# HAHHHD/mllp

Measured on AMD Instinct MI355X. Metric: LP instances/sec (fwd+bwd) on Netlib batch; achieved HBM GB/s on CSR SpMM, higher is better.
Workload: dtype f32; 1 GPU; netlib_full: BASELINE.json configs[2], 97 instances / 1,074,147 nnz per global batch, one block-diagonal batch per GPU, one Adam step per global batch: fwd + BCE + bwd + gradient all-reduce + Adam, fp32; global_batch=97, instances_rank0=97, nnz_rank0=1074147, hip_graph=False, parallelism=dp1

## Files before the change

### mllp_amd/csrc/fused_kernels.hip

```cpp
#include <algorithm>
#include <vector>

#include "device_utils.h"
#include "host_graph.h"
#include "internal.h"
#include "node_bodies.h"

namespace mllp {

typedef float f32x4m __attribute__((ext_vector_type(4)));

#ifdef MLLP_TIMING_BUILD
static int g_fused_abl = [] {
    const char* e = getenv("MLLP_FUSED_ABL");
    return e ? atoi(e) : 0;
}();
#define FUSED_ABL(bit) ((J.abl & (bit)) != 0)
__device__ unsigned long long g_fused_stamps[8192 * 8];
__device__ unsigned long long g_fused_stamps1[8192 * 8];
#define FUSED_STAMP(k)                                                                      \
    {                                                                                       \
        __builtin_amdgcn_sched_barrier(0);                                                  \
        const unsigned long long now_ = __builtin_amdgcn_s_memtime();                       \
        __builtin_amdgcn_sched_barrier(0);                                                  \
// ... 1293 lines not shown
    const int tid = threadIdx.x, lane = tid & 63, wave = tid >> 6;
    for (int j = 0; j < A.n_jobs; ++j) {
        const BwdJob1& J = A.job[j];
        BwdW1& W = Ws_[j];
        if (tid < 16) { W.wv[tid] = J.p.Wv[tid]; W.bv[tid] = J.p.bv[tid]; W.we[tid] = J.p.we[tid]; }
        if (tid == 0) { W.pq = J.D[OFF_PQ]; W.pq0 = J.D[OFF_PQ0]; W.pt = J.D[OFF_PT]; W.pt0 = J.D[OFF_PT0]; }
    }
    __syncthreads();
    float* tiles = tiles_ + wave * TILE1;
    const int px = blockIdx.x % NP, bi = blockIdx.x / NP, gp = gridDim.x / NP;
    const int gw = bi * FW + wave;
#ifdef MLLP_TIMING_BUILD
    unsigned long long stamp_sum[8] = {0, 0, 0, 0, 0, 0, 0, 0};
    unsigned long long stamp_last = __builtin_amdgcn_s_memtime();
    const unsigned long long stamp_begin = stamp_last;
#define STAMP_ARGS1 , stamp_sum, stamp_last
#else
#define STAMP_ARGS1
#endif
    for (int j = 0; j < A.n_jobs; ++j) {
        const BwdJob1& J = A.job[j];
        const PartTiers P = J.s.part[px];
        f32x4m accT = splat4(0.0f);
        float accS[6] = {0.0f, 0.0f, 0.0f, 0.0f, 0.0f, 0.0f};
        for (int k = bi; k < P.n_block; k += gp)
            bwd1_row(J, Ws_[j], block_slot<1>(J.s, P.row0 + k, tid), lane, merge_lds, tiles, accT, accS STAMP_ARGS1);
        WaveList wl = wave_list(J.s, px, gw);
        for (int c0 = 0; c0 < wl.L; c0 += 64) {
            wave_list_chunk(wl, c0, lane);
            int it = wave_list_get(wl, 0);
            SlotReq q = item_request<1>(J.s, P, max(it, 0), lane);
            for (int k = 0; it >= 0; ++k) {
                const int itn = wave_list_get(wl, k + 1);
                const RowSlot r = slot_make(q);
                q = item_request<1>(J.s, P, max(itn, 0), lane);
                bwd1_row(J, Ws_[j], r, lane, merge_lds, tiles, accT, accS STAMP_ARGS1);
#ifdef MLLP_TIMING_BUILD
                stamp_sum[7] += 1;
#endif
                it = itn;
            }
        }
        __syncthreads();
        float* red = tiles_;
#pragma unroll
        for (int q = 0; q < 4; ++q) red[wave * 262 + ((lane >> 4) * 4 + q) * 16 + (lane & 15)] = accT[q];
#pragma unroll
        for (int i = 0; i < 6; ++i) {
            const float v = wave_sum(accS[i]);
            if (lane == 0) red[wave * 262 + 256 + i] = v;
        }
        __syncthreads();
        float* dst = J.stats + (size_t)blockIdx.x * STAT_FLOATS;
        for (int i = tid; i < STAT_FLOATS; i += FT) dst[i] = 0.0f;
        __syncthreads();
        if (tid < 262) {
            float v = 0.0f;
            for (int w = 0; w < FW; ++w) v += red[w * 262 + tid];
            const int o = tid >> 4, n = tid & 15;
            if (tid >= 256) {
                const int i = tid - 256;
                const int slot = i == 0 ? 768 : i == 1 ? 1024 : i == 2 ? 1280 : i == 3 ? 1280 + 16 : i == 4 ? 1536 : 1536 + 16;
                dst[slot] = v;
            } else if (n == 0) dst[o * 16] = v;
            else if (n == 1) dst[256 + o * 16] = v;
            else if (n < 5) dst[512 + o * 16 + (n - 2)] = v;
        }
        __syncthreads();
#ifdef MLLP_TIMING_BUILD
        stamp_last = __builtin_amdgcn_s_memtime();
#endif
    }
#ifdef MLLP_TIMING_BUILD
    if (lane == 0) {
        stamp_sum[6] = __builtin_amdgcn_s_memtime() - stamp_begin;
        unsigned long long* d = g_fused_stamps1 + (size_t)(blockIdx.x * FW + wave) * 8;
        for (int k = 0; k < 8; ++k) d[k] = stamp_sum[k];
    }
#endif
#undef STAMP_ARGS1
}

__global__ __launch_bounds__(RT) void fused_head_bwd_kernel(int n, const float* __restrict__ h3, const float* __restrict__ fcw,
                                                            const float* __restrict__ dlogits, const int* __restrict__ perm,
                                                            float* __restrict__ dh3, float* __restrict__ head_part) {
    __shared__ float head_lds[(RT / 64) * 18];
    const int tid = threadIdx.x, lane = tid & 63, part = lane & 3;
    HeadAcc ha;
    ha.w = f4zero(); ha.b = 0.0f; ha.l = 0.0f;
    const float4 fw = ld4(fcw + 4 * part);
    for (int row = blockIdx.x * (RT / 4) + (tid >> 2); row < n; row += gridDim.x * (RT / 4)) {
        const float dz = dlogits[perm[row]];
        const float4 hv = ld4(h3 + (size_t)row * 16 + 4 * part);
        *reinterpret_cast<float4*>(dh3 + (size_t)row * 16 + 4 * part) = f4scale(fw, dz);
        fma4(dz, hv, ha.w);
        if (part == 0) ha.b += dz;
    }
    head_partials_store<RT / 64>(ha, head_lds, head_part, tid);
}

struct ReduceArgs {
    const float* stats[MODEL_CONVS];
    float* out[MODEL_CONVS];
    int nblk;
    const float* head_part;
    float* head_out;
    float* loss_out;
};

__device__ __forceinline__ void fused_reduce_body(const ReduceArgs& A, int n_conv) {
    __shared__ float sh[32][32];
    const int tid = threadIdx.x;
    if ((int)blockIdx.x == n_conv * STAT_TILES) {
        if (!A.head_part) return;
        const int col = tid & 31, slice = tid >> 5;
        float v = 0.0f;
        if (col < 18)
            for (int b = slice; b < A.nblk; b += 32) v += A.head_part[(size_t)b * 18 + col];
        sh[slice][col] = v;
        __syncthreads();
        if (tid < 18) {
            float t = 0.0f;
            for (int q = 0; q < 32; ++q) t += sh[q][tid];
            if (tid < 17) A.head_out[tid] = t;
            else if (A.loss_out) A.loss_out[0] = t;
        }
        return;
    }
    float* sh4 = &sh[0][0];
    const int col = tid & 255, slice = tid >> 8;
    const int c = blockIdx.x / STAT_TILES, tile = blockIdx.x % STAT_TILES;
    const float* src = A.stats[c] + tile * 256 + col;
    float v = 0.0f;
    int b = slice;
    for (; b + 124 < A.nblk; b += 128) {
        float t[32];
#pragma unroll
        for (int q = 0; q < 32; ++q) t[q] = src[(size_t)(b + 4 * q) * STAT_FLOATS];
#pragma unroll
        for (int q = 0; q < 32; ++q) v += t[q];
    }
    for (; b + 28 < A.nblk; b += 32) {
        float t[8];
#pragma unroll
        for (int q = 0; q < 8; ++q) t[q] = src[(size_t)(b + 4 * q) * STAT_FLOATS];
#pragma unroll
        for (int q = 0; q < 8; ++q) v += t[q];
    }
    for (; b < A.nblk; b += 4) v += src[(size_t)b * STAT_FLOATS];
    sh4[slice * 256 + col] = v;
    __syncthreads();
    if (tid < 256) A.out[c][tile * 256 + tid] = (sh4[tid] + sh4[256 + tid]) + (sh4[512 + tid] + sh4[768 + tid]);
}
__global__ __launch_bounds__(RT) void fused_reduce_kernel(ReduceArgs A, int n_conv) { fused_reduce_body(A, n_conv); }

struct TailArgs {
    ReduceArgs R;
    ConvParams p[MODEL_CONVS];
    int cin[MODEL_CONVS];
    float* grads[MODEL_CONVS];
    float* zero;
    int n_zero;
    float* params; const float* grads_all; float* m; float* v; float* state;
    float eps;
    int n_params;
    float* D[MODEL_CONVS];
    unsigned long long* sync;
    unsigned* err;
};
__device__ __forceinline__ bool tail_barrier(unsigned long long* cnt, unsigned long long target, unsigned* err_host) {
    __shared__ int ok_s;
    unsigned long long* err_dev = cnt + 2;
    __syncthreads();
    if (threadIdx.x == 0) {
        __threadfence();
        __hip_atomic_fetch_add(cnt, 1ull, __ATOMIC_RELEASE, __HIP_MEMORY_SCOPE_AGENT);
        int spins = 0;
        while (__hip_atomic_load(cnt, __ATOMIC_ACQUIRE, __HIP_MEMORY_SCOPE_AGENT) < target && ++spins < (1 << 22))
            __builtin_amdgcn_s_sleep(8);
        if (spins >= (1 << 22)) {
            __hip_atomic_store(err_dev, 1ull, __ATOMIC_RELAXED, __HIP_MEMORY_SCOPE_AGENT);
            __hip_atomic_store(err_host, 1u, __ATOMIC_RELAXED, __HIP_MEMORY_SCOPE_SYSTEM);
        }
        __threadfence();
        ok_s = __hip_atomic_load(err_dev, __ATOMIC_RELAXED, __HIP_MEMORY_SCOPE_AGENT) == 0ull;
    }
    __syncthreads();
    return ok_s != 0;
}
__global__ __launch_bounds__(RT) void fused_tail_kernel(TailArgs A, int n_conv) {
    const unsigned long long G = gridDim.x, epoch = A.sync[1];
    const int b = blockIdx.x;
    const float step = A.state[0] + 1.0f, lr = A.state[1], b1 = A.state[2], b2 = A.state[3];
    fused_reduce_body(A.R, n_conv);
    if (!tail_barrier(A.sync, (epoch + 1) * G, A.err)) return;
    if (b < n_conv) {
        finalize_conv_body(A.cin[b], A.p[b], A.R.out[b], 1, A.grads[b]);
        __syncthreads();
        const int off = (int)(A.grads[b] - A.grads_all), n = 4 * FEAT * A.cin[b] + 5 * FEAT;
        adam_slice(A.params + off, A.grads_all + off, A.m + off, A.v + off, step, lr, b1, b2, A.eps, 1.0f, n);
        __syncthreads();
        if (threadIdx.x < BLOCK) param_prep_body(A.p[b], A.cin[b], A.D[b]);
    } else if (b == n_conv) {
        for (int k = threadIdx.x; k < A.n_zero; k += RT) A.zero[k] = 0.0f;
        const int off = (int)(A.R.head_out - A.grads_all);
        adam_slice(A.params + off, A.grads_all + off, A.m + off, A.v + off, step, lr, b1, b2, A.eps, 1.0f, A.n_params - off);
        if (threadIdx.x == 0) {
            A.state[0] = step;
            A.sync[1] = epoch + 1;
        }
    }
}

__global__ __launch_bounds__(256) void fused_fill_kernel(int n_dst, const int* __restrict__ perm, const int* __restrict__ ptr,
                                                         const int* __restrict__ idx, const float* __restrict__ val,
                                                         const int* __restrict__ inv_src, const int* __restrict__ sptr,
                                                         int2* __restrict__ sent) {
    const int k = blockIdx.x * 4 + (threadIdx.x >> 6), lane = threadIdx.x & 63;
    if (k >= n_dst) return;
    const int r = perm[k], beg = ptr[r], deg = ptr[r + 1] - beg, o = sptr[k];
    for (int e = lane; e < deg; e += 64) sent[o + e] = make_int2(inv_src[idx[beg + e]], __float_as_int(val[beg + e]));
}
__global__ void fused_permute_kernel(int n, const int* __restrict__ perm, const float* __restrict__ src, float* __restrict__ dst) {
    for (int i = blockIdx.x * blockDim.x + threadIdx.x; i < n; i += gridDim.x * blockDim.x) dst[i] = src[perm[i]];
}
__global__ void fused_pregather_kernel(int64_t nnz, const int2* __restrict__ sent, const float* __restrict__ xs,
                                       float2* __restrict__ sax) {
    for (int64_t e = blockIdx.x * (int64_t)blockDim.x + threadIdx.x; e < nnz; e += (int64_t)gridDim.x * blockDim.x) {
        const int2 v = sent[e];
        sax[e] = make_float2(__int_as_float(v.y), xs[v.x]);
    }
}

#ifdef MLLP_TIMING_BUILD
extern "C" int mllp_timing_read_stamps(unsigned long long* host, int n) {
    return hipMemcpyFromSymbol(host, HIP_SYMBOL(g_fused_stamps), (size_t)n * sizeof(unsigned long long)) == hipSuccess ? 0 : -1;
}
extern "C" int mllp_timing_read_stamps1(unsigned long long* host, int n) {
    return hipMemcpyFromSymbol(host, HIP_SYMBOL(g_fused_stamps1), (size_t)n * sizeof(unsigned long long)) == hipSuccess ? 0 : -1;
}
#endif

template <class T>
static int dev_alloc(mllp_graph* g, size_t count, T** out, const T* host = nullptr, size_t room = 1) {
    void* p = nullptr;
    MLLP_HIP_TRY(hipMalloc(&p, std::max<size_t>(count, room) * sizeof(T)));
    if (count < room) MLLP_HIP_TRY(hipMemset(p, 0, room * sizeof(T)));
    g->allocs.push_back(p);
    if (host && count) MLLP_HIP_TRY(hipMemcpy(p, host, count * sizeof(T), hipMemcpyHostToDevice));
    *out = static_cast<T*>(p);
    return MLLP_OK;
}

static void set_tiers(FusedTiersDev& d, const FusedTiers& t) {
    d.n_block = t.n_block; d.n_wave = t.n_wave; d.n_group = t.n_group; d.n_base = t.n_base;
}

int fused_refill_values(mllp_graph* g, hipStream_t s) {
    int rc;
    if (g->M > 0) {
        hipLaunchKernelGGL(fused_fill_kernel, dim3((unsigned)((g->M + 3) / 4)), dim3(256), 0, s, (int)g->M, g->perm_c, g->A.ptr,
                           g->A.idx, g->A.val, g->inv_v, g->FA.sptr, reinterpret_cast<int2*>(g->FA.sent));
        if ((rc = check_launch("fused_fill A"))) return rc;
    }
    if (g->N > 0) {
        hipLaunchKernelGGL(fused_fill_kernel, dim3((unsigned)((g->N + 3) / 4)), dim3(256), 0, s, (int)g->N, g->perm_v, g->At.ptr,
                           g->At.idx, g->At.val, g->inv_c, g->FAt.sptr, reinterpret_cast<int2*>(g->FAt.sent));
        if ((rc = check_launch("fused_fill At"))) return rc;
    }
    return MLLP_OK;
}

int fused_graph_build(mllp_graph* g, const int* h_csr_ptr, const int* h_csc_ptr) {
    if (g->fused_built) return MLLP_OK;
    if ((int64_t)g->h_csr_ptr.size() != g->M + 1 && !h_csr_ptr) return fail(MLLP_EINVAL, "fused path: no host row pointers");
    HostFusedOrient hc, hv;
    {
#ifdef MLLP_SCALAR_PARTITION
        const std::vector<int> part = host_partition_instances(host_instance_cost(h_csr_ptr, g->h_inst_ptr_m),
                                                               host_instance_cost(h_csc_ptr, g->h_inst_ptr_n), FUSED_PARTS);
#else
        const std::vector<int> part = host_partition_instances_v(host_instance_loads(h_csr_ptr, g->h_inst_ptr_m),
                                                                 host_instance_loads(h_csc_ptr, g->h_inst_ptr_n), FUSED_PARTS);
#endif
        host_build_fused_orient(h_csr_ptr, (int)g->M, g->h_inst_ptr_m, part, &hc);
        host_build_fused_orient(h_csc_ptr, (int)g->N, g->h_inst_ptr_n, part, &hv);
    }
    int rc;
    if ((rc = dev_alloc(g, (size_t)g->M, &g->perm_c, hc.perm.data()))) return rc;
    if ((rc = dev_alloc(g, (size_t)g->N, &g->perm_v, hv.perm.data()))) return rc;
    if ((rc = dev_alloc(g, (size_t)g->M, &g->inv_c, hc.inv.data()))) return rc;
    if ((rc = dev_alloc(g, (size_t)g->N, &g->inv_v, hv.inv.data()))) return rc;
    FusedOrient& A = g->FA;
    FusedOrient& At = g->FAt;
    A.n_dst = (int)g->M; A.n_src = (int)g->N; A.nnz = (int)g->nnz;
    At.n_dst = (int)g->N; At.n_src = (int)g->M; At.nnz = (int)g->nnz;
    for (int q = 0; q < NP; ++q) {
        set_tiers(A.t16[q], hc.t16[q]); set_tiers(A.t1[q], hc.t1[q]);
        set_tiers(At.t16[q], hv.t16[q]); set_tiers(At.t1[q], hv.t1[q]);
    }
    for (int q = 0; q <= NP; ++q) { A.row0[q] = hc.row0[q]; At.row0[q] = hv.row0[q]; }
    {
        const int gp = fused_grid(g) / NP;
        const HostFusedOrient* ho[2] = {&hc, &hv};
        FusedOrient* dv[2] = {&A, &At};
        for (int k = 0; k < 2; ++k) {
            HostWaveLists l16, l16x2, l1;
            host_build_wave_lists(*ho[k], false, gp * FW, FW, 4, &l16);
            host_build_wave_lists(*ho[k], false, 2 * gp * FW, FW, 2, &l16x2);
            host_build_wave_lists(*ho[k], true, gp * FW, FW, 8, &l1);
            FusedOrient& d = *dv[k];
            d.L16 = l16.L; d.nw16 = l16.waves_per_part;
            d.L16x2 = l16x2.L; d.nw16x2 = l16x2.waves_per_part;
            d.L1 = l1.L; d.nw1 = l1.waves_per_part;
            if ((rc = dev_alloc(g, l16.order.size(), &d.lst16, l16.order.data()))) return rc;
            if ((rc = dev_alloc(g, l16x2.order.size(), &d.lst16x2, l16x2.order.data()))) return rc;
            if ((rc = dev_alloc(g, l1.order.size(), &d.lst1, l1.order.data()))) return rc;
        }
    }
    if ((rc = dev_alloc(g, (size_t)g->M + 1, &A.sptr, hc.sptr.data(), 2))) return rc;
    if ((rc = dev_alloc(g, (size_t)g->N + 1, &At.sptr, hv.sptr.data(), 2))) return rc;
    if ((rc = dev_alloc(g, (size_t)g->nnz * 2, &A.sent, (const int*)nullptr, 2))) return rc;
    if ((rc = dev_alloc(g, (size_t)g->nnz * 2, &At.sent, (const int*)nullptr, 2))) return rc;
    if ((rc = dev_alloc(g, (size_t)g->nnz * 2, &A.sax, (const float*)nullptr, 2))) return rc;
    if ((rc = dev_alloc(g, (size_t)g->nnz * 2, &At.sax, (const float*)nullptr, 2))) return rc;
    if ((rc = dev_alloc(g, (size_t)g->N, &g->inv_n_p))) return rc;
    if ((rc = dev_alloc(g, (size_t)g->N, &g->x1_p))) return rc;
    if ((rc = dev_alloc(g, (size_t)g->M, &g->x2_p))) return rc;
    if ((rc = dev_alloc(g, (size_t)g->N, &g->labels_p))) return rc;
    if (!g->tail_sync) {
        if ((rc = dev_alloc(g, (size_t)4, &g->tail_sync))) return rc;
        MLLP_HIP_TRY(hipMemset(g->tail_sync, 0, 32));
        MLLP_HIP_TRY(hipHostMalloc((void**)&g->tail_err_host, 64, hipHostMallocMapped));
        *g->tail_err_host = 0u;
        MLLP_HIP_TRY(hipHostGetDevicePointer((void**)&g->tail_err_dev, g->tail_err_host, 0));
    }
    if ((rc = fused_refill_values(g, 0))) return rc;
    if (g->N > 0) {
        hipLaunchKernelGGL(fused_permute_kernel, dim3(256), dim3(256), 0, 0, (int)g->N, g->perm_v, g->inv_n, g->inv_n_p);
        if ((rc = check_launch("fused_permute inv_n"))) return rc;
    }
    MLLP_HIP_TRY(hipDeviceSynchronize());
    g->fused_built = true;
    return MLLP_OK;
}

int fused_bind(mllp_graph* g, const float* x1, const float* x2, const float* labels, hipStream_t s) {
    int rc;
    hipStreamCaptureStatus cap = hipStreamCaptureStatusNone;
    (void)hipStreamIsCapturing(s, &cap);
    const bool capturing = cap != hipStreamCaptureStatusNone;
    if (capturing) g->bound_x1 = g->bound_x2 = g->bound_labels = nullptr;
    if (x1 != g->bound_x1 || x2 != g->bound_x2) {
        if (g->N > 0) hipLaunchKernelGGL(fused_permute_kernel, dim3(256), dim3(256), 0, s, (int)g->N, g->perm_v, x1, g->x1_p);
        if (g->M > 0) hipLaunchKernelGGL(fused_permute_kernel, dim3(256), dim3(256), 0, s, (int)g->M, g->perm_c, x2, g->x2_p);
        if (g->nnz > 0) {
            hipLaunchKernelGGL(fused_pregather_kernel, dim3(1024), dim3(256), 0, s, g->nnz,
                               reinterpret_cast<const int2*>(g->FA.sent), g->x1_p, reinterpret_cast<float2*>(g->FA.sax));
            hipLaunchKernelGGL(fused_pregather_kernel, dim3(1024), dim3(256), 0, s, g->nnz,
                               reinterpret_cast<const int2*>(g->FAt.sent), g->x2_p, reinterpret_cast<float2*>(g->FAt.sax));
        }
        if ((rc = check_launch("fused_bind inputs"))) return rc;
        if (!capturing) { g->bound_x1 = x1; g->bound_x2 = x2; }
    }
    if (labels && labels != g->bound_labels) {
        if (g->N > 0) hipLaunchKernelGGL(fused_permute_kernel, dim3(256), dim3(256), 0, s, (int)g->N, g->perm_v, labels, g->labels_p);
        if ((rc = check_launch("fused_bind labels"))) return rc;
        if (!capturing) g->bound_labels = labels;
    }
    return MLLP_OK;
}

int fused_grid(const mllp_graph* g) { return std::max(std::min(g->n_cu, STAT_BLOCKS_MAX) / NP, 1) * NP; }

static FwdJob16 fwd_job16(const FusedOrient& o, const FusedModel& m, int c, const float* x_src, const float* x_dst, float* h) {
    const ConvWs& w = m.w.c[c];
    FwdJob16 J = {};
    J.s = items_dev(o, 0);
    J.x_src = x_src; J.x_dst = x_dst; J.D = w.derived; J.p = conv_params_at(conv_at(m.P, c), MODEL_CONV[c].cin);
    J.h = h; J.Z = w.Z; J.aux = w.aux;
    J.head = 0;
#ifdef MLLP_TIMING_BUILD
    J.abl = g_fused_abl;
#endif
    return J;
}
static FwdJob1 fwd_job1(const FusedOrient& o, const FusedModel& m, int c, const float* x_dst, float* h) {
    const ConvWs& w = m.w.c[c];
    FwdJob1 J = {};
    J.s = items_dev(o, 1);
    J.x_dst = x_dst; J.D = w.derived; J.p = conv_params_at(conv_at(m.P, c), MODEL_CONV[c].cin);
    J.h = h; J.Z = w.Z; J.aux = w.aux;
    return J;
}

int fused_forward(mllp_graph* g, const FusedModel& m, int head_mode, hipStream_t s, bool skip_prep) {
    const int G = fused_grid(g);
    const ModelWs& w = m.w;
    int rc;
    if ((rc = fused_bind(g, m.x1, m.x2, head_mode == 2 ? m.labels : nullptr, s))) return rc;
    if (!skip_prep && (rc = model_param_prep(m.P, w, s))) return rc;
    {
        FwdLaunch1 L = {};
        L.n_jobs = 2;
        L.job[0] = fwd_job1(g->FAt, m, CONV_1V, g->x1_p, w.h1v);
        L.job[1] = fwd_job1(g->FA, m, CONV_1C, g->x2_p, w.h1c);
        hipLaunchKernelGGL(fused_fwd1_kernel, dim3(G), dim3(FT), 0, s, L);
        if ((rc = check_launch("fused_fwd1"))) return rc;
    }
    {
        FwdLaunch16 L = {};
        L.n_jobs = 2;
        L.job[0] = fwd_job16(g->FAt, m, CONV_2V, w.h1c, w.h1v, w.h2v);
        L.job[1] = fwd_job16(g->FA, m, CONV_2C, w.h1v, w.h1c, w.h2c);
        L.job[0].perm = g->perm_v; L.job[1].perm = g->perm_c;
        hipLaunchKernelGGL(fused_fwd16_kernel, dim3(G), dim3(FT), 0, s, L);
        if ((rc = check_launch("fused_fwd16 layer 2"))) return rc;
    }
    {
        FwdLaunch16 L = {};
        L.n_jobs = 1;
        L.job[0] = fwd_job16(g->FAt, m, CONV_3V, w.h2c, w.h2v, w.h3v);
        FwdJob16& J = L.job[0];
        J.head = head_mode;
        J.fcw = m.P + OFF_FC; J.fcb = m.P + OFF_FC + FEAT; J.inv_n = g->inv_n_p; J.labels = g->labels_p; J.perm = g->perm_v;
        J.inv_batch = m.inv_batch;
        J.logits = m.logits; J.g_out = w.d3v; J.head_part = w.head_partials;
        hipLaunchKernelGGL(fused_fwd16_kernel, dim3(G), dim3(FT), 0, s, L);
        if ((rc = check_launch("fused_fwd16 layer 3"))) return rc;
    }
    return MLLP_OK;
}

int fused_head_backward(const mllp_graph* g, const FusedModel& m, const float* dlogits, hipStream_t s) {
    const int G = fused_grid(g);
    hipLaunchKernelGGL(fused_head_bwd_kernel, dim3(G), dim3(RT), 0, s, (int)g->N, m.w.h3v, m.P + OFF_FC, dlogits, g->perm_v,
                       m.w.d3v, m.w.head_partials);
    return check_launch("fused_head_bwd");
}

static BwdJob16 bwd_job16(const FusedOrient& o, const FusedModel& m, int c, const float* x_src, const float* x_dst,
                          const float* h, const float* dh_a, const float* dh_b, float* dx_dst, bool need_rec, bool mask_dx) {
    const ConvWs& w = m.w.c[c];
    BwdJob16 J = {};
    J.s = items_dev(o, 0);
    J.x_src = x_src; J.x_dst = x_dst; J.D = w.derived; J.p = conv_params_at(conv_at(m.P, c), MODEL_CONV[c].cin);
    J.h = h; J.dh_a = dh_a; J.dh_b = dh_b; J.Z = w.Z; J.aux = w.aux;
    J.rec = need_rec ? w.rec : nullptr;
    J.dx_dst = dx_dst;
    J.mask_dx = mask_dx ? 1 : 0;
    J.stats = w.stats;
#ifdef MLLP_TIMING_BUILD
    J.abl = g_fused_abl;
#endif
    return J;
}
static SrcJob16 src_job16(const FusedOrient& o_src_major, const ConvWs& w, const float* x_rows, float* dx, const float* add) {
    SrcJob16 J = {};
    J.s = items_dev(o_src_major, 2);
    J.x = x_rows; J.rec = w.rec; J.dx = dx;
    J.addp = add ? add : x_rows; J.addw = add ? 1.0f : 0.0f; J.mask = 1;
    return J;
}
static BwdJob1 bwd_job1(const FusedOrient& o, const FusedModel& m, int c, const float* x_dst, const float* g_masked) {
    const ConvWs& w = m.w.c[c];
    BwdJob1 J = {};
    J.s = items_dev(o, 1);
    J.x_dst = x_dst; J.D = w.derived; J.p = conv_params_at(conv_at(m.P, c), MODEL_CONV[c].cin);
    J.g = g_masked; J.Z = w.Z; J.aux = w.aux; J.stats = w.stats;
    return J;
}

int fused_backward(const mllp_graph* g, const FusedModel& m, bool premasked, float* grads, float* loss, hipStream_t s,
                   const FusedAdam* adam) {
    const int G = fused_grid(g);
    const ModelWs& w = m.w;
    int rc;
    const FusedOrient& A = g->FA;
    const FusedOrient& At = g->FAt;
    {
        BwdLaunch16 L = {};
        L.n_jobs = 1;
        L.job[0] = bwd_job16(At, m, CONV_3V, w.h2c, w.h2v, premasked ? nullptr : w.h3v, w.d3v, nullptr, w.d2v, true, true);
        hipLaunchKernelGGL(fused_bwd16_kernel, dim3(G), dim3(FT), 0, s, L);
        if ((rc = check_launch("fused_bwd16 C3"))) return rc;
    }
    {
        SrcLaunch16 S = {};
        S.n_jobs = 1;
        S.job[0] = src_job16(A, w.c[CONV_3V], w.h2c, w.d2c, nullptr);
        hipLaunchKernelGGL(fused_src16_kernel, dim3(2 * G), dim3(FT), 0, s, S);
        if ((rc = check_launch("fused_src16 C3"))) return rc;
        BwdLaunch16 L = {};
        L.n_jobs = 1;
        L.job[0] = bwd_job16(At, m, CONV_2V, w.h1c, w.h1v, nullptr, w.d2v, nullptr, w.d1v, true, true);
        hipLaunchKernelGGL(fused_bwd16_kernel, dim3(G), dim3(FT), 0, s, L);
        if ((rc = check_launch("fused_bwd16 C2V"))) return rc;
    }
    {
        BwdLaunch16 L = {};
        L.n_jobs = 1;
        L.job[0] = bwd_job16(A, m, CONV_2C, w.h1v, w.h1c, nullptr, w.d2c, nullptr, w.d1c, true, true);
        hipLaunchKernelGGL(fused_bwd16_kernel, dim3(G), dim3(FT), 0, s, L);
        if ((rc = check_launch("fused_bwd16 C2C"))) return rc;
        SrcLaunch16 S = {};
        S.n_jobs = 2;
        S.job[0] = src_job16(A, w.c[CONV_2V], w.h1c, w.d1c_b, w.d1c);
        S.job[1] = src_job16(At, w.c[CONV_2C], w.h1v, w.d1v_b, w.d1v);
        hipLaunchKernelGGL(fused_src16_kernel, dim3(2 * G), dim3(FT), 0, s, S);
        if ((rc = check_launch("fused_src16 C2V + C2C"))) return rc;
    }
    {
        BwdLaunch1 L = {};
        L.n_jobs = 2;
        L.job[0] = bwd_job1(A, m, CONV_1C, g->x2_p, w.d1c_b);
        L.job[1] = bwd_job1(At, m, CONV_1V, g->x1_p, w.d1v_b);
        hipLaunchKernelGGL(fused_bwd1_kernel, dim3(G), dim3(FT), 0, s, L);
        if ((rc = check_launch("fused_bwd1"))) return rc;
    }
    ReduceArgs R = {};
    for (int c = 0; c < MODEL_CONVS; ++c) { R.stats[c] = w.c[c].stats; R.out[c] = w.c[c].red; }
    R.nblk = G;
    R.head_part = w.head_partials;
    R.head_out = grads + OFF_FC;
    R.loss_out = loss;
    if (adam) {
        TailArgs T = {};
        T.R = R;
        for (int c = 0; c < MODEL_CONVS; ++c) {
            T.p[c] = conv_params_at(conv_at(m.P, c), MODEL_CONV[c].cin);
            T.cin[c] = MODEL_CONV[c].cin;
            T.grads[c] = conv_at(grads, c);
            T.D[c] = w.c[c].derived;
        }
        T.zero = grads + OFF_UNUSED;
        T.n_zero = LEN_UNUSED;
        T.params = adam->params; T.grads_all = grads; T.m = adam->m; T.v = adam->v; T.state = adam->state;
        T.eps = adam->eps;
        T.n_params = adam->n;
        T.sync = g->tail_sync;
        T.err = g->tail_err_dev;
        if (g->tail_err_host && *(volatile unsigned*)g->tail_err_host != 0u)
            return fail(MLLP_EHIP, "the grid barrier of fused_tail_kernel timed out in an earlier step (the device was shared with "
                                   "other work): parameters and optimizer state since then are invalid; recreate the graph");
        hipLaunchKernelGGL(fused_tail_kernel, dim3(MODEL_CONVS * STAT_TILES + 1), dim3(RT), 0, s, T, MODEL_CONVS);
        return check_launch("fused_tail");
    }
    {
        hipLaunchKernelGGL(fused_reduce_kernel, dim3(MODEL_CONVS * STAT_TILES + 1), dim3(RT), 0, s, R, MODEL_CONVS);
        if ((rc = check_launch("fused_reduce"))) return rc;
    }
    return model_finalize(g, m.P, w, true, grads, s);
}

}
```

### mllp_amd/csrc/host_graph.cpp

```cpp
#include "host_graph.h"

#include <array>

#include <algorithm>
#include <atomic>
#include <thread>

#include "../../include/mllp_hip.h"

namespace mllp {

int host_build_batch(int64_t n_inst, const int64_t* inst_m, const int64_t* inst_n, const int64_t* indptr,
                     const int32_t* indices, const double* values, HostBatch* out, std::string* err,
                     unsigned max_threads) {
    auto bad_arg = [&](int code, const char* msg) {
        if (err) *err = msg;
        return code;
    };
    if (!out) return bad_arg(MLLP_EINVAL, "host_build_batch: out is null");
    if (n_inst < 0 || (n_inst > 0 && (!inst_m || !inst_n || !indptr)))
        return bad_arg(MLLP_EINVAL, "mllp_graph_create_host: null instance arrays");
    std::vector<int64_t> pm(n_inst + 1, 0), pn(n_inst + 1, 0), pe(n_inst + 1, 0), pp(n_inst + 1, 0);
    for (int64_t k = 0; k < n_inst; ++k) {
        if (inst_m[k] < 0 || inst_n[k] < 0) return bad_arg(MLLP_EINVAL, "negative instance size");
// ... 23 lines not shown
            if (k >= n_inst || bad.load()) break;
            const int64_t m = inst_m[k], n = inst_n[k], e0 = pe[k], e1 = pe[k + 1];
            const int64_t* ip = indptr + pp[k];
            const int32_t* ix = indices + e0;
            const double* va = values + e0;
            cnt.assign(n + 1, 0);
            bool ok = true;
            for (int64_t r = 0; r < m && ok; ++r) {
                if (ip[r + 1] < ip[r] || ip[r + 1] > e1 - e0) { bad = 1; ok = false; break; }
                b.csr_ptr[pm[k] + r + 1] = (int)(e0 + ip[r + 1]);
                int prev = -1;
                for (int64_t e = ip[r]; e < ip[r + 1]; ++e) {
                    const int c = ix[e];
                    if (c < 0 || c >= n || c <= prev) { bad = 2; ok = false; break; }
                    prev = c;
                    b.csr_idx[e0 + e] = (int)(pn[k] + c);
                    b.csr_val[e0 + e] = (float)va[e];
                    cnt[c + 1]++;
                }
            }
            if (!ok) break;
            for (int64_t c = 0; c < n; ++c) cnt[c + 1] += cnt[c];
            for (int64_t c = 0; c < n; ++c) b.csc_ptr[pn[k] + c + 1] = (int)(e0 + cnt[c + 1]);
            for (int64_t r = 0; r < m; ++r)
                for (int64_t e = ip[r]; e < ip[r + 1]; ++e) {
                    const int c = ix[e];
                    const int64_t pos = e0 + cnt[c]++;
                    b.csc_idx[pos] = (int)(pm[k] + r);
                    b.csc_val[pos] = (float)va[e];
                }
        }
    };
    unsigned nt = max_threads ? max_threads : std::max(1u, std::min(16u, std::thread::hardware_concurrency()));
    nt = (unsigned)std::min<int64_t>(nt, std::max<int64_t>(n_inst, 1));
    std::vector<std::thread> th;
    for (unsigned i = 1; i < nt; ++i) th.emplace_back(worker);
    worker();
    for (auto& t : th) t.join();
    if (bad == 1) return bad_arg(MLLP_EINVAL, "indptr not monotone");
    if (bad == 2) return bad_arg(MLLP_EINVAL, "column ids must be in range, sorted and unique within a row");
    b.pm = std::move(pm);
    b.pn = std::move(pn);
    return MLLP_OK;
}

TierConfig host_choose_tiers(int64_t nnz, int tier_wave, int tier_block) {
    const bool throughput = nnz >= (int64_t)32 << 20;
    TierConfig c;
    c.tier_wave = tier_wave > 0 ? tier_wave : (throughput ? 1024 : 64);
    c.tier_block = tier_block > 0 ? tier_block : (throughput ? 16384 : 256);
    if (c.tier_block < c.tier_wave) c.tier_block = c.tier_wave;
    c.chunk_nnz = 4 * c.tier_block;
    return c;
}

void host_build_tiers(const int* ptr, int n_dst, const TierConfig& cfg, HostTiers* out) {
    HostTiers& t = *out;
    t = HostTiers();
    int slots = 0;
    for (int r = 0; r < n_dst; ++r) {
        const int beg = ptr[r], end = ptr[r + 1], deg = end - beg;
        if (deg > cfg.tier_block) {
            const int nck = (deg + cfg.chunk_nnz - 1) / cfg.chunk_nnz;
            if (nck == 1) {
                t.chunks.insert(t.chunks.end(), {r, beg, end, -1});
            } else {
                t.split.insert(t.split.end(), {r, slots, nck, 0});
                const int per = ((deg + nck - 1) / nck + 255) & ~255;
                for (int c = 0; c < nck; ++c) {
                    const int cb = std::min(beg + c * per, end), ce = std::min(cb + per, end);
                    t.chunks.insert(t.chunks.end(), {r, cb, ce, slots++});
                }
            }
        } else if (deg > cfg.tier_wave) {
            t.rows_wave.push_back(r);
        } else {
            t.n_group++;
        }
    }
    t.n_slots = slots;
    t.short_rows = n_dst > 0 && (double)ptr[n_dst] / n_dst <= 16.0;
}

std::vector<int64_t> host_instance_cost(const int* ptr, const std::vector<int64_t>& inst_off) {
    constexpr int64_t ITEM = FUSED_COST_ITEM, STEP = FUSED_COST_STEP;
    const size_t n = inst_off.empty() ? 0 : inst_off.size() - 1;
    std::vector<int64_t> cost(n, 0);
    for (size_t k = 0; k < n; ++k) {
        int64_t c = 0;
        for (int64_t r = inst_off[k]; r < inst_off[k + 1]; ++r) {
            const int64_t deg = ptr[r + 1] - ptr[r];
            if (deg > FUSED_T16[2]) c += 12 * FUSED_COST_BLOCK_ROW;
            else if (deg > FUSED_T16[1]) c += ITEM + STEP * ((deg + 63) / 64);
            else if (deg > FUSED_T16[0]) c += (ITEM + STEP * ((deg + 15) / 16)) / 4;
            else c += (ITEM + STEP * ((deg + 3) / 4)) / 16;
        }
        cost[k] = c;
    }
    return cost;
}

std::vector<InstLoad> host_instance_loads(const int* ptr, const std::vector<int64_t>& inst_off) {
    const size_t n = inst_off.empty() ? 0 : inst_off.size() - 1;
    std::vector<InstLoad> out(n);
    for (size_t k = 0; k < n; ++k) {
        InstLoad& l = out[k];
        for (int64_t r = inst_off[k]; r < inst_off[k + 1]; ++r) {
            const int64_t deg = ptr[r + 1] - ptr[r];
            if (deg > FUSED_T16[2]) { l.d[0] += 16 * FUSED_BLOCK_ROW_ITEMS; l.d[1] += 16 * 2 * ((deg + 767) / 768); l.d[4] += 1; }
            else if (deg > FUSED_T16[1]) { l.d[0] += 16; l.d[1] += 16 * ((deg + 63) / 64); }
            else if (deg > FUSED_T16[0]) { l.d[0] += 4; l.d[1] += 4 * ((deg + 15) / 16); }
            else { l.d[0] += 1; l.d[1] += std::max<int64_t>((deg + 3) / 4, 1); }
            if (deg > FUSED_T1[2]) { l.d[2] += 64 * FUSED_BLOCK_ROW_ITEMS; l.d[3] += 64 * 2 * ((deg + 6143) / 6144); }
            else if (deg > FUSED_T1[1]) { l.d[2] += 64; l.d[3] += 64 * ((deg + 511) / 512); }
            else if (deg > FUSED_T1[0]) { l.d[2] += 4; l.d[3] += 4 * ((deg + 31) / 32); }
            else { l.d[2] += 1; l.d[3] += std::max<int64_t>((deg + 7) / 8, 1); }
            if (deg > FUSED_T16[2]) l.d[5] += 12 * FUSED_COST_BLOCK_ROW;
            else if (deg > FUSED_T16[1]) l.d[5] += FUSED_COST_ITEM + FUSED_COST_STEP * ((deg + 63) / 64);
            else if (deg > FUSED_T16[0]) l.d[5] += (FUSED_COST_ITEM + FUSED_COST_STEP * ((deg + 15) / 16)) / 4;
            else l.d[5] += (FUSED_COST_ITEM + FUSED_COST_STEP * ((deg + 3) / 4)) / 16;
        }
    }
    return out;
}

namespace {
struct VecBalance {
    static constexpr int D = 2 * FUSED_LOAD_DIMS;
    int n_parts;
    std::vector<std::array<double, D>> x;
    std::vector<std::array<double, D>> load;
    double max_of(int q) const {
        double m = 0.0;
        for (int d = 0; d < D; ++d) m = std::max(m, load[(size_t)q][d]);
        return m;
    }
    double worst() const {
        double m = 0.0;
        for (int q = 0; q < n_parts; ++q) m = std::max(m, max_of(q));
        return m;
    }
};
}

double host_partition_imbalance(const std::vector<InstLoad>& a, const std::vector<InstLoad>& b, const std::vector<int>& part,
                                int n_parts) {
    double worst = 0.0;
    for (int side = 0; side < 2; ++side)
        for (int d = 0; d < FUSED_LOAD_DIMS; ++d) {
            if (d == 4) continue;
            std::vector<double> l((size_t)n_parts, 0.0);
            double tot = 0.0;
            for (size_t i = 0; i < a.size(); ++i) {
                const double v = (double)(side ? b[i].d[d] : a[i].d[d]);
                l[(size_t)part[i]] += v;
                tot += v;
            }
            if (tot <= 0.0) continue;
            for (int q = 0; q < n_parts; ++q) worst = std::max(worst, l[(size_t)q] * n_parts / tot);
        }
    return worst;
}

std::vector<int> host_partition_instances_v(const std::vector<InstLoad>& a, const std::vector<InstLoad>& b, int n_parts) {
    const int n = (int)a.size();
    constexpr int D = VecBalance::D;
    VecBalance vb;
    vb.n_parts = n_parts;
    vb.x.assign((size_t)n, std::array<double, D>{});
    vb.load.assign((size_t)n_parts, std::array<double, D>{});
    double tot[D] = {};
    for (int i = 0; i < n; ++i)
        for (int d = 0; d < FUSED_LOAD_DIMS; ++d) { tot[d] += (double)a[i].d[d]; tot[FUSED_LOAD_DIMS + d] += (double)b[i].d[d]; }
    std::vector<double> size((size_t)n, 0.0);
    for (int i = 0; i < n; ++i)
        for (int d = 0; d < D; ++d) {
            const double v = (double)(d < FUSED_LOAD_DIMS ? a[i].d[d] : b[i].d[d - FUSED_LOAD_DIMS]);
            vb.x[(size_t)i][d] = tot[d] > 0.0 && d % FUSED_LOAD_DIMS != 4 ? v * n_parts / tot[d] : 0.0;
            size[(size_t)i] = std::max(size[(size_t)i], vb.x[(size_t)i][d]);
        }
    std::vector<int> order((size_t)n), part((size_t)n, 0);
    for (int i = 0; i < n; ++i) order[(size_t)i] = i;
    std::stable_sort(order.begin(), order.end(), [&](int p, int q) { return size[(size_t)p] > size[(size_t)q]; });
    std::vector<int> count((size_t)n_parts, 0);
    for (int i : order) {
        int best = 0;
        double best_v = 0.0;
        for (int q = 0; q < n_parts; ++q) {
            double v = 0.0;
            for (int d = 0; d < D; ++d) v = std::max(v, vb.load[(size_t)q][d] + vb.x[(size_t)i][d]);
            if (q == 0 || v < best_v - 1e-12 || (v < best_v + 1e-12 && count[(size_t)q] < count[(size_t)best])) { best = q; best_v = v; }
        }
        part[(size_t)i] = best;
        count[(size_t)best]++;
        for (int d = 0; d < D; ++d) vb.load[(size_t)best][d] += vb.x[(size_t)i][d];
    }
    if (n <= 4096) {
        for (int round = 0; round < 200; ++round) {
            int wq = 0;
            for (int q = 1; q < n_parts; ++q)
                if (vb.max_of(q) > vb.max_of(wq)) wq = q;
            const double cur = vb.max_of(wq);
            double best_gain = 1e-9;
            int bi = -1, bj = -1, bq = -1;
            auto pair_max = [&](int q1, int q2, int i, int j) {
                double m = 0.0;
                for (int d = 0; d < D; ++d) {
                    const double xi = vb.x[(size_t)i][d], xj = j >= 0 ? vb.x[(size_t)j][d] : 0.0;
                    m = std::max(m, std::max(vb.load[(size_t)q1][d] - xi + xj, vb.load[(size_t)q2][d] + xi - xj));
                }
                return m;
            };
            for (int i = 0; i < n; ++i) {
                if (part[(size_t)i] != wq) continue;
                for (int q = 0; q < n_parts; ++q) {
                    if (q == wq) continue;
                    const double m0 = pair_max(wq, q, i, -1);
                    if (cur - m0 > best_gain) { best_gain = cur - m0; bi = i; bj = -1; bq = q; }
                    for (int j = 0; j < n; ++j) {
                        if (part[(size_t)j] != q) continue;
                        const double m1 = pair_max(wq, q, i, j);
                        if (cur - m1 > best_gain) { best_gain = cur - m1; bi = i; bj = j; bq = q; }
                    }
                }
            }
            if (bi < 0) break;
            for (int d = 0; d < D; ++d) {
                const double xi = vb.x[(size_t)bi][d], xj = bj >= 0 ? vb.x[(size_t)bj][d] : 0.0;
                vb.load[(size_t)wq][d] += xj - xi;
                vb.load[(size_t)bq][d] += xi - xj;
            }
            part[(size_t)bi] = bq;
            if (bj >= 0) part[(size_t)bj] = wq;
        }
    }
    std::vector<int64_t> ca((size_t)n), cb((size_t)n);
    for (int i = 0; i < n; ++i) { ca[(size_t)i] = a[(size_t)i].d[5]; cb[(size_t)i] = b[(size_t)i].d[5]; }
    const std::vector<int> alt = host_partition_instances(ca, cb, n_parts);
    return host_partition_imbalance(a, b, alt, n_parts) < host_partition_imbalance(a, b, part, n_parts) - 1e-12 ? alt : part;
}

std::vector<int> host_partition_instances(const std::vector<int64_t>& cost_a, const std::vector<int64_t>& cost_b, int n_parts) {
    const int n = (int)cost_a.size();
    std::vector<int64_t> ca((size_t)n), cb((size_t)n);
    int64_t sa = 1, sb = 1;
    for (int i = 0; i < n; ++i) {
        ca[i] = cost_a[i] + 1;
        cb[i] = cost_b[i] + 1;
        sa += ca[i]; sb += cb[i];
    }
    std::vector<int> order((size_t)n), part((size_t)n, 0);
    for (int i = 0; i < n; ++i) order[i] = i;
    std::stable_sort(order.begin(), order.end(), [&](int a, int b) { return ca[a] + cb[a] > ca[b] + cb[b]; });
    std::vector<int64_t> la((size_t)n_parts, 0), lb((size_t)n_parts, 0);
    for (int i : order) {
        int best = 0;
        double best_v = 0.0;
        for (int q = 0; q < n_parts; ++q) {
            const double v = std::max((double)(la[q] + ca[i]) / (double)sa, (double)(lb[q] + cb[i]) / (double)sb);
            if (q == 0 || v < best_v) { best = q; best_v = v; }
        }
        part[i] = best;
        la[best] += ca[i];
        lb[best] += cb[i];
    }
    return part;
}

void host_build_fused_orient(const int* ptr, int n, const std::vector<int64_t>& inst_off, const std::vector<int>& inst_part,
                             HostFusedOrient* out) {
    HostFusedOrient& o = *out;
    o = HostFusedOrient();
    n = std::max(n, 0);
    o.perm.resize((size_t)n);
    o.inv.resize((size_t)n);
    o.sptr.assign((size_t)n + 1, 0);
    std::vector<int> node_part((size_t)n, 0);
    for (size_t k = 0; k + 1 < inst_off.size(); ++k)
        for (int64_t r = inst_off[k]; r < inst_off[k + 1] && r < n; ++r) node_part[(size_t)r] = inst_part[k];
    for (int r = 0; r < n; ++r) o.perm[r] = r;
    std::stable_sort(o.perm.begin(), o.perm.end(), [&](int a, int b) {
        if (node_part[a] != node_part[b]) return node_part[a] < node_part[b];
        return ptr[a + 1] - ptr[a] > ptr[b + 1] - ptr[b];
    });
    for (int q = 0; q <= FUSED_PARTS; ++q) o.row0[q] = 0;
    for (int k = 0; k < n; ++k) {
        const int r = o.perm[k], deg = ptr[r + 1] - ptr[r], q = node_part[r];
        o.inv[r] = k;
        o.sptr[k + 1] = o.sptr[k] + deg;
        o.row0[q + 1]++;
        for (int which = 0; which < 2; ++which) {
            const int(&T)[3] = which ? FUSED_T1 : FUSED_T16;
            FusedTiers& t = which ? o.t1[q] : o.t16[q];
            if (deg > T[2]) t.n_block++;
            else if (deg > T[1]) t.n_wave++;
            else if (deg > T[0]) t.n_group++;
            else t.n_base++;
        }
    }
    for (int q = 0; q < FUSED_PARTS; ++q) o.row0[q + 1] += o.row0[q];
}

void host_build_wave_lists(const HostFusedOrient& o, bool scalar, int waves_per_part, int waves_per_wg, int nnz_per_step,
                           HostWaveLists* out) {
    HostWaveLists& wl = *out;
    wl = HostWaveLists();
    const int nw = std::max(waves_per_part, 1), wpg = std::max(std::min(waves_per_wg, nw), 1), gp = std::max(nw / wpg, 1);
    wl.waves_per_part = nw;
    const int U = scalar ? 64 : 16, RG = U / 4;
    const int e_base = std::max(nnz_per_step, 1), e_group = 4 * e_base, e_wave = (scalar ? 64 : 16) * e_base;
    std::vector<std::vector<int>> lists((size_t)FUSED_PARTS * nw);
    for (int q = 0; q < FUSED_PARTS; ++q) {
        const FusedTiers& t = scalar ? o.t1[q] : o.t16[q];
        const int n_gitems = (t.n_group + RG - 1) / RG, n_bitems = (t.n_base + U - 1) / U;
        const int n_items = t.n_wave + n_gitems + n_bitems;
        auto deg_of = [&](int rl) { const int k = o.row0[q] + rl; return (int64_t)o.sptr[(size_t)k + 1] - o.sptr[(size_t)k]; };
        std::vector<std::pair<int64_t, int>> items((size_t)n_items);
        for (int it = 0; it < n_items; ++it) {
            int64_t steps;
            if (it < t.n_wave) steps = (deg_of(t.n_block + it) + e_wave - 1) / e_wave;
            else if (it < t.n_wave + n_gitems) steps = (deg_of(t.n_block + t.n_wave + (it - t.n_wave) * RG) + e_group - 1) / e_group;
            else steps = (deg_of(t.n_block + t.n_wave + t.n_group + (it - t.n_wave - n_gitems) * U) + e_base - 1) / e_base;
            items[(size_t)it] = {FUSED_COST_ITEM + FUSED_COST_STEP * std::max<int64_t>(steps, 1), it};
        }
        std::stable_sort(items.begin(), items.end(), [](const auto& a, const auto& b) { return a.first > b.first; });
        std::vector<int64_t> load((size_t)nw, 0), slow((size_t)nw, 0);
        for (int w = 0; w < nw; ++w) {
            const int bi = w / wpg;
            const int n_rows = bi < gp && t.n_block > bi ? (t.n_block - bi + gp - 1) / gp : 0;
            slow[(size_t)w] = 1000 + 95 * ((w % wpg) / 4);
            load[(size_t)w] = FUSED_COST_BLOCK_ROW * n_rows * slow[(size_t)w] / 1000;
        }
        for (const auto& itc : items) {
            int best = 0;
            int64_t best_t = 0;
            for (int w = 0; w < nw; ++w) {
                const int64_t tw = load[(size_t)w] + itc.first * slow[(size_t)w] / 1000;
                if (w == 0 || tw < best_t) { best = w; best_t = tw; }
            }
            lists[(size_t)q * nw + best].push_back(itc.second);
            load[(size_t)best] = best_t;
        }
        for (int w = 0; w < nw; ++w) {
            wl.max_load = std::max(wl.max_load, load[(size_t)w]);
            wl.sum_load += load[(size_t)w];
            wl.L = std::max(wl.L, (int)lists[(size_t)q * nw + w].size());
        }
    }
    wl.L = std::max(wl.L, 1);
    wl.order.assign((size_t)FUSED_PARTS * nw * wl.L, -1);
    for (size_t k = 0; k < lists.size(); ++k) std::copy(lists[k].begin(), lists[k].end(), wl.order.begin() + k * wl.L);
}

}
```

### mllp_amd/csrc/host_graph.h

```cpp
#pragma once
#include <stdint.h>

#include <string>
#include <vector>

namespace mllp {

struct HostBatch {
    int64_t M = 0, N = 0, nnz = 0, n_inst = 0;
    std::vector<int64_t> pm, pn;
    std::vector<int> csr_ptr, csr_idx;
    std::vector<float> csr_val;
    std::vector<int> csc_ptr, csc_idx;
    std::vector<float> csc_val;
};

int host_build_batch(int64_t n_inst, const int64_t* inst_m, const int64_t* inst_n, const int64_t* indptr,
                     const int32_t* indices, const double* values, HostBatch* out, std::string* err,
                     unsigned max_threads = 0);

struct TierConfig {
    int tier_wave = 0, tier_block = 0, chunk_nnz = 0;
};
TierConfig host_choose_tiers(int64_t nnz, int tier_wave, int tier_block);

struct HostTiers {
    std::vector<int> rows_wave;
    std::vector<int> chunks;
    std::vector<int> split;
    int n_group = 0, n_slots = 0;
    bool short_rows = false;
};
void host_build_tiers(const int* ptr, int n_dst, const TierConfig& cfg, HostTiers* out);

constexpr int FUSED_PARTS = 8;
struct FusedTiers {
    int n_block = 0, n_wave = 0, n_group = 0, n_base = 0;
};
struct HostFusedOrient {
    std::vector<int> perm;
    std::vector<int> inv;
    std::vector<int> sptr;
    int row0[FUSED_PARTS + 1];
    FusedTiers t16[FUSED_PARTS], t1[FUSED_PARTS];
};
constexpr int FUSED_T16[3] = {16, 64, 1024};
constexpr int FUSED_T1[3] = {16, 64, 4096};
constexpr int64_t FUSED_COST_ITEM = 5300, FUSED_COST_STEP = 2000, FUSED_COST_BLOCK_ROW = 25000;
std::vector<int64_t> host_instance_cost(const int* ptr, const std::vector<int64_t>& inst_off);
std::vector<int> host_partition_instances(const std::vector<int64_t>& cost_a, const std::vector<int64_t>& cost_b, int n_parts);
constexpr int FUSED_BLOCK_ROW_ITEMS = 10;
constexpr int FUSED_LOAD_DIMS = 6;
struct InstLoad {
    int64_t d[FUSED_LOAD_DIMS] = {0, 0, 0, 0, 0, 0};
};
std::vector<InstLoad> host_instance_loads(const int* ptr, const std::vector<int64_t>& inst_off);
std::vector<int> host_partition_instances_v(const std::vector<InstLoad>& a, const std::vector<InstLoad>& b, int n_parts);
double host_partition_imbalance(const std::vector<InstLoad>& a, const std::vector<InstLoad>& b, const std::vector<int>& part,
                                int n_parts);
void host_build_fused_orient(const int* ptr, int n, const std::vector<int64_t>& inst_off, const std::vector<int>& inst_part,
                             HostFusedOrient* out);
struct HostWaveLists {
    std::vector<int> order;
    int L = 0, waves_per_part = 0;
    int64_t max_load = 0, sum_load = 0;
};
void host_build_wave_lists(const HostFusedOrient& o, bool scalar, int waves_per_part, int waves_per_wg, int nnz_per_step,
                           HostWaveLists* out);

}
```

Baseline: 290,400 instances/s.

## Merge C2V and C2C bwd16 launches and precharge wave lists for sequential jobs

The separate C2V and C2C backward kernels now run as one two-job fused_bwd16 launch, which saves a kernel launch and a grid-wide boundary. The wave-list builder gains an optional initial-load vector. The second orientation's work is dealt so that waves that finish the first job late get less follow-on work, using per-workgroup finish times from the first job. Schedules are built both with and without this precharge and the one with the lower modeled makespan is kept. This adds host-side preprocessing complexity and relies on the cost model matching device timing.

```diff
diff --git a/mllp_amd/csrc/fused_kernels.hip b/mllp_amd/csrc/fused_kernels.hip
--- a/mllp_amd/csrc/fused_kernels.hip
+++ b/mllp_amd/csrc/fused_kernels.hip
@@ -1619,11 +1619,17 @@
     for (int q = 0; q <= NP; ++q) { A.row0[q] = hc.row0[q]; At.row0[q] = hv.row0[q]; }
     {
         const int gp = fused_grid(g) / NP;
-        const HostFusedOrient* ho[2] = {&hc, &hv};
-        FusedOrient* dv[2] = {&A, &At};
+        const HostFusedOrient* ho[2] = {&hv, &hc};
+        FusedOrient* dv[2] = {&At, &A};
+        std::vector<int64_t> first16;
         for (int k = 0; k < 2; ++k) {
             HostWaveLists l16, l16x2, l1;
+#ifdef MLLP_NO_PRECHARGE
             host_build_wave_lists(*ho[k], false, gp * FW, FW, 4, &l16);
+#else
+            host_build_wave_lists(*ho[k], false, gp * FW, FW, 4, &l16, k == 1 ? &first16 : nullptr);
+#endif
+            if (k == 0) first16 = host_workgroup_finish(l16, FW);
             host_build_wave_lists(*ho[k], false, 2 * gp * FW, FW, 2, &l16x2);
             host_build_wave_lists(*ho[k], true, gp * FW, FW, 8, &l1);
             FusedOrient& d = *dv[k];
@@ -1808,18 +1814,21 @@
         S.job[0] = src_job16(A, w.c[CONV_3V], w.h2c, w.d2c, nullptr);
         hipLaunchKernelGGL(fused_src16_kernel, dim3(2 * G), dim3(FT), 0, s, S);
         if ((rc = check_launch("fused_src16 C3"))) return rc;
-        BwdLaunch16 L = {};
-        L.n_jobs = 1;
-        L.job[0] = bwd_job16(At, m, CONV_2V, w.h1c, w.h1v, nullptr, w.d2v, nullptr, w.d1v, true, true);
-        hipLaunchKernelGGL(fused_bwd16_kernel, dim3(G), dim3(FT), 0, s, L);
-        if ((rc = check_launch("fused_bwd16 C2V"))) return rc;
     }
     {
         BwdLaunch16 L = {};
-        L.n_jobs = 1;
+        L.n_jobs = 2;
+#ifdef MLLP_BWD16_C2C_FIRST
+        L.job[1] = bwd_job16(At, m, CONV_2V, w.h1c, w.h1v, nullptr, w.d2v, nullptr, w.d1v, true, true);
         L.job[0] = bwd_job16(A, m, CONV_2C, w.h1v, w.h1c, nullptr, w.d2c, nullptr, w.d1c, true, true);
+#else
+        L.job[0] = bwd_job16(At, m, CONV_2V, w.h1c, w.h1v, nullptr, w.d2v, nullptr, w.d1v, true, true);
+        L.job[1] = bwd_job16(A, m, CONV_2C, w.h1v, w.h1c, nullptr, w.d2c, nullptr, w.d1c, true, true);
+#endif
         hipLaunchKernelGGL(fused_bwd16_kernel, dim3(G), dim3(FT), 0, s, L);
-        if ((rc = check_launch("fused_bwd16 C2C"))) return rc;
+        if ((rc = check_launch("fused_bwd16 C2V + C2C"))) return rc;
+    }
+    {
         SrcLaunch16 S = {};
         S.n_jobs = 2;
         S.job[0] = src_job16(A, w.c[CONV_2V], w.h1c, w.d1c_b, w.d1c);
diff --git a/mllp_amd/csrc/host_graph.cpp b/mllp_amd/csrc/host_graph.cpp
--- a/mllp_amd/csrc/host_graph.cpp
+++ b/mllp_amd/csrc/host_graph.cpp
@@ -349,14 +349,20 @@
 }
 
 void host_build_wave_lists(const HostFusedOrient& o, bool scalar, int waves_per_part, int waves_per_wg, int nnz_per_step,
-                           HostWaveLists* out) {
+                           HostWaveLists* out, const std::vector<int64_t>* initial_load) {
     HostWaveLists& wl = *out;
     wl = HostWaveLists();
     const int nw = std::max(waves_per_part, 1), wpg = std::max(std::min(waves_per_wg, nw), 1), gp = std::max(nw / wpg, 1);
     wl.waves_per_part = nw;
+    const bool charged = initial_load && !initial_load->empty();
+    auto init_of = [&](int q, int w) {
+        const size_t k = (size_t)q * nw + w;
+        return charged && k < initial_load->size() ? (*initial_load)[k] : (int64_t)0;
+    };
     const int U = scalar ? 64 : 16, RG = U / 4;
     const int e_base = std::max(nnz_per_step, 1), e_group = 4 * e_base, e_wave = (scalar ? 64 : 16) * e_base;
     std::vector<std::vector<int>> lists((size_t)FUSED_PARTS * nw);
+    wl.finish.assign((size_t)FUSED_PARTS * nw, 0);
     for (int q = 0; q < FUSED_PARTS; ++q) {
         const FusedTiers& t = scalar ? o.t1[q] : o.t16[q];
         const int n_gitems = (t.n_group + RG - 1) / RG, n_bitems = (t.n_base + U - 1) / U;
@@ -371,27 +377,50 @@
             items[(size_t)it] = {FUSED_COST_ITEM + FUSED_COST_STEP * std::max<int64_t>(steps, 1), it};
         }
         std::stable_sort(items.begin(), items.end(), [](const auto& a, const auto& b) { return a.first > b.first; });
-        std::vector<int64_t> load((size_t)nw, 0), slow((size_t)nw, 0);
+        auto deal = [&](bool with_init, std::vector<std::vector<int>>& ls, std::vector<int64_t>& load) {
+            std::vector<int64_t> slow((size_t)nw, 0);
+            ls.assign((size_t)nw, std::vector<int>());
+            load.assign((size_t)nw, 0);
+            for (int w = 0; w < nw; ++w) {
+                const int bi = w / wpg;
+                const int n_rows = bi < gp && t.n_block > bi ? (t.n_block - bi + gp - 1) / gp : 0;
+                slow[(size_t)w] = 1000 + 95 * ((w % wpg) / 4);
+                load[(size_t)w] = (with_init ? init_of(q, w) : 0) + FUSED_COST_BLOCK_ROW * n_rows * slow[(size_t)w] / 1000;
+            }
+            for (const auto& itc : items) {
+                int best = 0;
+                int64_t best_t = 0;
+                for (int w = 0; w < nw; ++w) {
+                    const int64_t tw = load[(size_t)w] + itc.first * slow[(size_t)w] / 1000;
+                    if (w == 0 || tw < best_t) { best = w; best_t = tw; }
+                }
+                ls[(size_t)best].push_back(itc.second);
+                load[(size_t)best] = best_t;
+            }
+            if (with_init)
+                for (int w = 0; w < nw; ++w) load[(size_t)w] -= init_of(q, w);
+        };
+        std::vector<std::vector<int>> ls;
+        std::vector<int64_t> load;
+        deal(false, ls, load);
+        if (charged) {
+            std::vector<std::vector<int>> lc;
+            std::vector<int64_t> loadc;
+            deal(true, lc, loadc);
+            int64_t fin = 0, finc = 0;
+            for (int w = 0; w < nw; ++w) {
+                fin = std::max(fin, init_of(q, w) + load[(size_t)w]);
+                finc = std::max(finc, init_of(q, w) + loadc[(size_t)w]);
+            }
+            if (finc < fin) { ls.swap(lc); load.swap(loadc); }
+        }
         for (int w = 0; w < nw; ++w) {
-            const int bi = w / wpg;
-            const int n_rows = bi < gp && t.n_block > bi ? (t.n_block - bi + gp - 1) / gp : 0;
-            slow[(size_t)w] = 1000 + 95 * ((w % wpg) / 4);
-            load[(size_t)w] = FUSED_COST_BLOCK_ROW * n_rows * slow[(size_t)w] / 1000;
-        }
-        for (const auto& itc : items) {
-            int best = 0;
-            int64_t best_t = 0;
-            for (int w = 0; w < nw; ++w) {
-                const int64_t tw = load[(size_t)w] + itc.first * slow[(size_t)w] / 1000;
-                if (w == 0 || tw < best_t) { best = w; best_t = tw; }
-            }
-            lists[(size_t)q * nw + best].push_back(itc.second);
-            load[(size_t)best] = best_t;
-        }
-        for (int w = 0; w < nw; ++w) {
-            wl.max_load = std::max(wl.max_load, load[(size_t)w]);
-            wl.sum_load += load[(size_t)w];
-            wl.L = std::max(wl.L, (int)lists[(size_t)q * nw + w].size());
+            const int64_t f = init_of(q, w) + load[(size_t)w];
+            wl.finish[(size_t)q * nw + w] = f;
+            wl.max_load = std::max(wl.max_load, f);
+            wl.sum_load += f;
+            wl.L = std::max(wl.L, (int)ls[(size_t)w].size());
+            lists[(size_t)q * nw + w].swap(ls[(size_t)w]);
         }
     }
     wl.L = std::max(wl.L, 1);
@@ -399,4 +428,17 @@
     for (size_t k = 0; k < lists.size(); ++k) std::copy(lists[k].begin(), lists[k].end(), wl.order.begin() + k * wl.L);
 }
 
-}
+std::vector<int64_t> host_workgroup_finish(const HostWaveLists& first, int waves_per_wg) {
+    const int nw = std::max(first.waves_per_part, 1), wpg = std::max(std::min(waves_per_wg, nw), 1);
+    std::vector<int64_t> out(first.finish.size(), 0);
+    for (int q = 0; q < FUSED_PARTS && (size_t)(q + 1) * nw <= first.finish.size(); ++q)
+        for (int w0 = 0; w0 < nw; w0 += wpg) {
+            const int w1 = std::min(w0 + wpg, nw);
+            int64_t m = 0;
+            for (int w = w0; w < w1; ++w) m = std::max(m, first.finish[(size_t)q * nw + w]);
+            for (int w = w0; w < w1; ++w) out[(size_t)q * nw + w] = m;
+        }
+    return out;
+}
+
+}
diff --git a/mllp_amd/csrc/host_graph.h b/mllp_amd/csrc/host_graph.h
--- a/mllp_amd/csrc/host_graph.h
+++ b/mllp_amd/csrc/host_graph.h
@@ -64,8 +64,10 @@
     std::vector<int> order;
     int L = 0, waves_per_part = 0;
     int64_t max_load = 0, sum_load = 0;
+    std::vector<int64_t> finish;
 };
 void host_build_wave_lists(const HostFusedOrient& o, bool scalar, int waves_per_part, int waves_per_wg, int nnz_per_step,
-                           HostWaveLists* out);
+                           HostWaveLists* out, const std::vector<int64_t>* initial_load = nullptr);
+std::vector<int64_t> host_workgroup_finish(const HostWaveLists& first, int waves_per_wg);
 
 }
```

After: 292,900 instances/s, median of 6. No clear change (+0.9%).
